# google-deepmind/dm_control

Hardware: AMD Instinct MI355X
Metric: env-steps/s (whole node) at batch 4096; max rel qpos error vs CPU (higher is better)
Workload: dtype f32

## Files before the change

### dm_control_amd/csrc/dmc_api.hip

```cpp
#include <hip/hip_runtime.h>
#include <dlfcn.h>

#include <cstdio>
#include <cstdlib>
#include <cstring>
#include <algorithm>
#include <string>
#include <type_traits>
#include <vector>

#include "../../include/dmc_batch.h"
#include "step_kernel.hip.h"
#include "step_tables.h"

namespace dmc {
hipError_t launch_step_f32(const LaunchGeom& g, hipStream_t stream, const StepLayout* d_layout, const StepOpts<float>& o,
                           const int* g_mi, const float* g_mr, const int* g_mc, const StepIO<float>& io, int nstep, int legacy, int mode, int outmask, int nsub);
hipError_t launch_step_f64(const LaunchGeom& g, hipStream_t stream, const StepLayout* d_layout, const StepOpts<double>& o,
                           const int* g_mi, const double* g_mr, const int* g_mc, const StepIO<double>& io, int nstep, int legacy, int mode, int outmask, int nsub);
}

using namespace dmc;

static thread_local std::string g_err;
// ... 257 lines not shown
      if (step_tables_build(&def, m->hm, nconmax, njmax, &err, njcon, -1)) {
        StepTables keep = b->tb; LaunchGeom kg = b->geom;
        b->tb = def;
        const bool def_fits = choose_geometry(b, lanes_per_env) == 0;
        if (fits && (!def_fits || b->geom.static_id < 0)) { b->tb = keep; b->geom = kg; }
      } else if (!fits) return fail(err);
    }
  }
  if (choose_geometry(b, lanes_per_env)) return -1;
  const StepLayout& L = b->tb.L;
  const StepDims& d = L.d;
  if (dev_alloc(b, &b->d_mi, (size_t)L.n_mi * sizeof(int), false, "") || dev_alloc(b, &b->d_mc, b->tb.mc.size() * sizeof(int), false, "") ||
      dev_alloc(b, &b->d_mr, (size_t)L.n_mr * b->elem, false, "") || dev_alloc(b, &b->d_layout, sizeof(StepLayout), false, "", &L)) return -2;
  if (upload_tables(b)) return -2;
  b->tb.opts.g_mr = b->d_mr;
  if (d.nslip) {
    if (dev_alloc(b, &b->d_ns_A, (size_t)b->B * d.nslip * d.nslip * b->elem, false, "noslip matrix")) return -2;
    b->tb.opts.ns_A = b->d_ns_A;
  }
  const int one = 1;
  if (dev_alloc(b, &b->d_epoch, sizeof(int), false, "stash epoch", &one)) return -2;
  if (dev_alloc(b, &b->d_work, 32 * 9 * sizeof(int), true, "work queue")) return -2;
  if (!getenv("DMC_NO_KSTASH") && !d.nmocap) {
    const size_t nk = (size_t)d.nq + d.nv + (L.s_qM - L.s_xpos);
    if (dev_alloc(b, &b->d_kstash, (size_t)b->B * nk * b->elem, false, "kinematic stash") ||
        dev_alloc(b, &b->d_kstash_i, (size_t)b->B * sizeof(int), true, "kinematic stash")) return -2;
  }
  if (b->geom.queue) {
    const int nit = (b->B * b->geom.lpe + 63) / 64;
    b->nxcd = getenv("DMC_XCDS") ? std::max(1, std::min(8, atoi(getenv("DMC_XCDS")))) : (b->ncu == 256 ? 8 : 1);
    if (b->geom.grid < 8 * b->nxcd) b->nxcd = 1;
    const bool one_l2_per_queue = b->nxcd > 1 || b->ncu <= 40 || getenv("DMC_XCDS");
    b->max_slices = getenv("DMC_SLICES") ? atoi(getenv("DMC_SLICES")) : (one_l2_per_queue ? 8 : 1);
    auto hw = [&](int n) { return b->precision == 64 ? n : (n + 1) / 2; };
    b->hand_n = hw(d.nq) + 2 * hw(d.nv) + hw(d.na) + 1;
    if (dev_alloc(b, &b->d_prog, (size_t)nit * sizeof(int), true, "piece counters") ||
        dev_alloc(b, &b->d_hand, (size_t)b->B * b->hand_n * sizeof(unsigned long long), false, "piece counters")) return -2;
  }
  if (b->geom.queue && !getenv("DMC_NO_LPT")) {
    b->nitems = (b->B * b->geom.lpe + 63) / 64;
    if (dev_alloc(b, &b->d_cost, (size_t)b->nitems * sizeof(int), true, "schedule") ||
        dev_alloc(b, &b->d_order, (size_t)b->nitems * sizeof(int), false, "schedule")) return -2;
    b->lpt = 1;
  }
  if (L.n_gs) {
    if (dev_alloc(b, &b->d_gscr, (size_t)b->B * L.n_gs * b->elem, true, "global scratch")) return -2;
    b->tb.opts.gscr = b->d_gscr;
// ... 101 lines not shown
    typedef int (*fn_t)(const LaunchGeom*, void*, const StepLayout*, const StepOpts<T>*, const int*, const T*, const int*, const StepIO<T>*, int, int, int, int, int);
    e = (hipError_t)((fn_t)b->spec_launch)(&b->geom, stream, b->d_layout, o, b->d_mi, (const T*)b->d_mr, b->d_mc, &io, nstep, legacy, mode, b->outmask, nsub);
  } else if constexpr (f64) e = launch_step_f64(b->geom, (hipStream_t)stream, b->d_layout, *o, b->d_mi, (const T*)b->d_mr, b->d_mc, io, nstep, legacy, mode, b->outmask, nsub);
  else e = launch_step_f32(b->geom, (hipStream_t)stream, b->d_layout, *o, b->d_mi, (const T*)b->d_mr, b->d_mc, io, nstep, legacy, mode, b->outmask, nsub);
  if (e != hipSuccess) return fail(std::string("kernel launch: ") + hipGetErrorString(e), -2);
  return 0;
}
static int launch_untimed(dmc_batch* b, int nstep, int legacy, LaunchMode mode, void* stream, const SeqArgs* sq) {
  HIP_TRY(hipSetDevice(b->device));
  b->launched_mask = b->outmask;
  return b->precision == 64 ? launch_t<double>(b, nstep, legacy, mode, stream, sq) : launch_t<float>(b, nstep, legacy, mode, stream, sq);
}
static int launch(dmc_batch* b, int nstep, int legacy, LaunchMode mode, void* stream, const SeqArgs* sq = nullptr) {
  HIP_TRY(hipSetDevice(b->device));
  TimerPair t;
  const bool timed = prof_begin(b, (hipStream_t)stream, &t);
  const int rc = launch_untimed(b, nstep, legacy, mode, stream, sq);
  const bool fwd = mode == MODE_FORWARD || mode == MODE_FORWARD_NOACT;
  if (timed) prof_end(b, (hipStream_t)stream, t, fwd ? 1 : 0,
                      mode == MODE_STEP ? nstep : mode == MODE_ROLLOUT ? nstep * (sq ? sq->nsub : 1) : mode == MODE_STEP1 ? 0 : 1);
  return rc;
}

extern "C" int dmc_batch_attach_specialised(dmc_batch* b, const char* so_path) {
  if (!b || !so_path) return fail("null argument");
  void* h = dlopen(so_path, RTLD_NOW | RTLD_LOCAL);
  if (!h) return fail(std::string("cannot load ") + so_path + ": " + dlerror());
  typedef const StepLayout* (*layout_t)();
  typedef void (*info_t)(int*);
  layout_t fl = (layout_t)dlsym(h, "dmc_spec_layout");
  info_t fi = (info_t)dlsym(h, "dmc_spec_info");
  void* launch = dlsym(h, "dmc_spec_launch");
  if (!fl || !fi || !launch) { dlclose(h); return fail("not a specialisation plugin (dmc_spec_* symbols missing)"); }
  int info[8]; fi(info);
  if (info[4] != b->precision) { dlclose(h); return fail("the plugin was built for another precision"); }
  const int so = b->precision == 64 ? (int)sizeof(StepOpts<double>) : (int)sizeof(StepOpts<float>);
  const int sio = b->precision == 64 ? (int)sizeof(StepIO<double>) : (int)sizeof(StepIO<float>);
  if (info[0] != (int)sizeof(StepLayout) || info[1] != so || info[2] != sio || info[3] != DMC_MODEL_VERSION || info[7] != (int)sizeof(LaunchGeom)) {
    dlclose(h); return fail("the plugin was built from other sources than this library (struct sizes / model version differ)");
  }
  if (info[5] != b->geom.lpe) { dlclose(h); return fail("the plugin was built for another lanes-per-environment shape"); }
  if (memcmp(fl(), &b->tb.L, sizeof(StepLayout)) != 0) { dlclose(h); return fail("the plugin's layout is not this batch's (another model or other caps)"); }
  if (b->spec_so) dlclose(b->spec_so);
  b->spec_so = h; b->spec_launch = launch; b->spec_features = info[6];
  typedef int (*tb_t)();
  tb_t tb = (tb_t)dlsym(h, "dmc_spec_task_args_bytes");
  b->spec_task_bytes = tb ? tb() : 0;
  b->task_on = 0;
  return 0;
}

extern "C" int dmc_batch_set_task_args(dmc_batch* b, const void* args, int nbytes) {
  if (!b || !args) return fail("null argument");
  if (!b->spec_task_bytes) return fail("the batch's kernel carries no task epilogue (attach a plugin built with a task header)");
  if (nbytes != b->spec_task_bytes) return fail("task argument block: size differs from the one the kernel was generated with");
  HIP_TRY(hipSetDevice(b->device));
  if (!b->d_task_args && dev_alloc(b, &b->d_task_args, (size_t)nbytes, false, "task arguments")) return -2;
  HIP_TRY(hipMemcpy(b->d_task_args, args, (size_t)nbytes, hipMemcpyHostToDevice));
  return 0;
}
extern "C" int dmc_batch_enable_task(dmc_batch* b, int on) {
  if (!b) return fail("null batch");
  if (on && (!b->spec_task_bytes || !b->d_task_args)) return fail("no task epilogue to enable (dmc_batch_set_task_args first)");
  b->task_on = on ? 1 : 0;
  return 0;
}

extern "C" int dmc_batch_step(dmc_batch* b, int nstep, int legacy_step, void* hip_stream) {
  if (!b) return fail("null batch");
  if (nstep < 1) return fail("nstep must be >= 1");
  if (legacy_step == 2 && b->tb.opts.integrator == DMC_INT_RK4) return fail("legacy_step 2 (step + mj_forward) is not implemented for RK4 models");
  return launch(b, nstep, legacy_step == 2 ? 2 : (legacy_step ? 1 : 0), MODE_STEP, hip_stream);
// ... 1091 lines not shown
```

### dm_control_amd/csrc/step_core.h

```cpp
#pragma once
#include "../../include/dmc_model_layout.h"
#include "step_layout.h"
#include "step_defs.h"
#include "step_math.h"
#include "step_lanes.h"
#include "step_dense.h"
#include "step_geom.h"

namespace dmc {
#ifdef DMC_HOST_EMU
inline int& emu_split_solves() { static int n = 0; return n; }
inline long long* emu_ls_counts() { static long long n[6] = {0, 0, 0, 0, 0, 0}; return n; }
inline long long* emu_ls_passes() { static long long n[3] = {0, 0, 0}; return n; }
#endif

#if defined(DMC_PROFILE) && !defined(DMC_HOST_EMU)
#define DMC_PROF(id) do { if (lane == 0) { const int t_ = (int)__builtin_readcyclecounter(); SI(prof)[id] += t_ - SI(prof)[33]; SI(prof)[33] = t_; } } while (0)
#else
#define DMC_PROF(id) ((void)0)
#endif
#ifdef DMC_TRACE_SUB
#define DMC_TSUB(region, cond, row) do { if (DMC_TRACE_SUB == (region) && (cond)) sub_stamp(row); } while (0)
#else
#define DMC_TSUB(region, cond, row) ((void)0)
// ... 225 lines not shown
      else __hip_atomic_store((unsigned*)(io.ctrl + (size_t)i*B + env), __float_as_uint((float)S(ctrl)[i]), __ATOMIC_RELAXED, __HIP_MEMORY_SCOPE_AGENT);
    }
  }
  DMC_DEV void load_handoff(const StepIO<T>& io, int env) {
    env = late(env);
    const int nq = L.d.nq, nv = L.d.nv, na = L.d.na, B = io.B;
    const u64h* h = io.hand + (size_t)env * io.hand_n;
    hand_get(S(qpos), h, nq); h += hand_words(nq);
    hand_get(S(qvel), h, nv); h += hand_words(nv);
    hand_get(S(qacc_warmstart), h, nv); h += hand_words(nv);
    if (na) { hand_get(S(act), h, na); h += hand_words(na); FOR_LANES(i, na) S(act_dot)[i] = 0; }
    { const u64h w = __hip_atomic_load(h, __ATOMIC_RELAXED, __HIP_MEMORY_SCOPE_AGENT); double t; __builtin_memcpy(&t, &w, 8); time_ = t; }
    FOR_LANES(i, nv) S(qfrc_applied)[i] = io.qfrc_applied ? io.qfrc_applied[(size_t)i*B + env] : (T)0;
    FOR_LANES(i, L.d.nu) {
      if (sizeof(T) == 8) { const u64h w = __hip_atomic_load((const u64h*)(io.ctrl + (size_t)i*B + env), __ATOMIC_RELAXED, __HIP_MEMORY_SCOPE_AGENT); T v; __builtin_memcpy(&v, &w, 8); S(ctrl)[i] = v; }
      else S(ctrl)[i] = (T)__uint_as_float(__hip_atomic_load((const unsigned*)(io.ctrl + (size_t)i*B + env), __ATOMIC_RELAXED, __HIP_MEMORY_SCOPE_AGENT));
    }
  }
#else
  DMC_DEV void store_handoff(const StepIO<T>&, int) {}
  DMC_DEV void load_handoff(const StepIO<T>&, int) {}
#endif
  DMC_DEV int kin_count() const { return L.s_qM - L.s_xpos; }
  DMC_DEV bool load_kstash(const StepIO<T>& io, int env) {
    env = late(env);
    if (io.kstash_i[env] != get_epoch()) return false;
    const int nq = L.d.nq, nv = L.d.nv, nk = kin_count();
    const T* h = io.kstash + (size_t)env*(nq + nv + nk);
    int bad = 0;
    FOR_LANES(i, nq) if (!(h[i] == S(qpos)[i])) bad = 1;
    FOR_LANES(i, nv) if (!(h[nq + i] == S(qvel)[i])) bad = 1;
    if (group_max<LPE>(bad)) return false;
    FOR_LANES(i, nk) S(xpos)[i] = h[nq + nv + i];
    DMC_WSYNC();
    kstash_env_geoms();
    return true;
  }
  DMC_DEV void store_kstash(const StepIO<T>& io, int env) {
    env = late(env);
    const int nq = L.d.nq, nv = L.d.nv, nk = kin_count();
    DMC_GLB T* h = G(io.kstash) + (size_t)env*(nq + nv + nk);
    FOR_LANES(i, nq) h[i] = S(qpos)[i];
    FOR_LANES(i, nv) h[nq + i] = S(qvel)[i];
    FOR_LANES(i, nk) h[nq + nv + i] = S(xpos)[i];
    if (lane == 0) G(io.kstash_i)[env] = get_epoch();
  }
  static constexpr bool kFeat = LS::kNV <= 0 || DMC_STATIC_FEATURES;
  static constexpr bool kSlices = LS::kNV <= 0 || LS::kNV > 16;
  static constexpr int kPFKin = LS::kNKin > 0 ? ((LS::kNKin + LPE - 1) / LPE < 24 ? (LS::kNKin + LPE - 1) / LPE : 24) : 0;
  struct Entry { int em, fast, kvalid, epoch; };
  struct EntryRegs {
    T qpos, qvel, warm, qfrc, ctrl, act, kq, kv;
    int ktag, epoch;
    T kd[kPFKin ? kPFKin : 1];
  };
  DMC_DEV static bool kstash_applies(const StepOpts<T>& o, const StepIO<T>& io, int mode, int legacy) {
    return io.kstash && mode == 0 && legacy && o.integrator != DMC_INT_RK4 && !io.stash_r;
  }
  DMC_DEV static void entry_issue(const StepLayout& L, const StepOpts<T>& o, const StepIO<T>& io, int env, int lane, int mode,
                                  int legacy, Entry* e, EntryRegs* r) {
    e->em = io.env_mode ? io.env_mode[env] : 0;
    e->kvalid = 0;
    e->epoch = *io.epoch;
#ifdef DMC_HOST_EMU
    e->fast = 0;
#else
    e->fast = (L.d.nq <= LPE && L.d.nv <= LPE && L.d.nu <= LPE && L.d.na <= LPE && !io.stash_r) ? 1 : 0;
#endif
    r->ktag = 0; r->epoch = 1;
    if (!e->fast) return;
    const size_t B = (size_t)io.B;
    const int nq = L.d.nq, nv = L.d.nv;
    r->qpos = lane < nq ? G(io.qpos)[lane*B + env] : (T)0;
    r->qvel = lane < nv ? G(io.qvel)[lane*B + env] : (T)0;
    r->warm = lane < nv ? G(io.qacc_warmstart)[lane*B + env] : (T)0;
    r->qfrc = (io.qfrc_applied && lane < nv) ? G(io.qfrc_applied)[lane*B + env] : (T)0;
    r->ctrl = lane < L.d.nu ? G(io.ctrl)[lane*B + env] : (T)0;
    r->act = (L.d.na && lane < L.d.na) ? G(io.act)[lane*B + env] : (T)0;
    if (!kstash_applies(o, io, mode, legacy)) return;
    r->ktag = G(io.kstash_i)[env]; r->epoch = e->epoch;
    const int nk = L.s_qM - L.s_xpos;
    const DMC_GLB T* h = G(io.kstash) + (size_t)env*(nq + nv + nk);
    r->kq = lane < nq ? h[lane] : (T)0;
    r->kv = lane < nv ? h[nq + lane] : (T)0;
#pragma unroll
    for (int k = 0; k < kPFKin; k++) { const int i = lane + k*LPE; r->kd[k] = i < nk ? h[nq + nv + i] : (T)0; }
  }
  DMC_DEV static void entry_commit(const StepLayout& L, const StepIO<T>& io, int env, int lane, Entry* e, const EntryRegs& r, T* s) {
    if (!e->fast) return;
    const int nq = L.d.nq, nv = L.d.nv;
    if (lane < nq) s[L.s_qpos + lane] = r.qpos;
    if (lane < nv) { s[L.s_qvel + lane] = r.qvel; s[L.s_qacc_warmstart + lane] = r.warm; s[L.s_qfrc_applied + lane] = r.qfrc; }
    if (lane < L.d.nu) s[L.s_ctrl + lane] = r.ctrl;
    if (L.d.na && lane < L.d.na) s[L.s_act + lane] = r.act;
    if (r.ktag != r.epoch) return;
    const int bad = ((lane < nq && !(r.kq == r.qpos)) || (lane < nv && !(r.kv == r.qvel))) ? 1 : 0;
    if (group_max<LPE>(bad)) return;
    const int nk = L.s_qM - L.s_xpos;
#pragma unroll
    for (int k = 0; k < kPFKin; k++) { const int i = lane + k*LPE; if (i < nk) s[L.s_xpos + i] = r.kd[k]; }
    if (kPFKin*LPE < nk) {
      const T* h = io.kstash + (size_t)env*(nq + nv + nk) + nq + nv;
      for (int i = lane + kPFKin*LPE; i < nk; i += LPE) s[L.s_xpos + i] = h[i];
    }
    e->kvalid = 1;
  }
  DMC_DEV void kstash_env_geoms() {
    if (!o.eg_n) return;
    FOR_LANES(g, L.d.ngeom) {
      const int k = o.eg_slot[g];
      if (k < 0) continue;
      const T* eg = (const T*)o.eg_data + (size_t)16*k*o.eg_B + SI(imisc)[IM_ENV];
      for (int j = 0; j < 3; j++) S(geom_xpos)[3*g + j] = eg[(size_t)j*o.eg_B];
      for (int j = 0; j < 9; j++) SG(geom_xmat)[9*g + j] = eg[(size_t)(3 + j)*o.eg_B];
    }
    DMC_WSYNC();
  }
  DMC_DEV void load_state(const StepIO<T>& io, int env, bool have_stash, const Entry& en, bool from_hand = false) {
    const int B = io.B;
    if (kSlices && from_hand) load_handoff(io, env);
    else if (en.fast) {
      if (L.d.na && lane < L.d.na) S(act_dot)[lane] = 0;
      time_ = io.time[env];
    } else {
      FOR_LANES(i, L.d.nq) S(qpos)[i] = io.qpos[(size_t)i*B + env];
      FOR_LANES(i, L.d.nv) {
        S(qvel)[i] = io.qvel[(size_t)i*B + env];
// ... 4 lines not shown
      if (L.d.na) FOR_LANES(i, L.d.na) { S(act)[i] = io.act[(size_t)i*B + env]; S(act_dot)[i] = 0; }
      time_ = io.time[env];
    }
    if (lane == 0) SI(imisc)[IM_ENV] = env;
    if (have_stash) {
      if (LPE >= 16) { if (lane < DMC_NWARNING) SI(imisc)[IM_WARN + lane] = 0; } else if (lane == 0) for (int k = 0; k < DMC_NWARNING; k++) SI(imisc)[IM_WARN + k] = 0;
      DMC_WSYNC();
      return;
    }
    if (lane == 0) {
      for (int k = 0; k < DMC_NWARNING; k++) SI(imisc)[IM_WARN + k] = 0;
      SI(imisc)[IM_NCON] = 0; SI(imisc)[IM_NEFC] = 0; SI(imisc)[IM_ITER] = 0;
      T* xp = S(xpos); T* xq = SG(xquat); T* xm = S(xmat); T* xi = S(xipos);
      xp[0] = xp[1] = xp[2] = 0; xi[0] = xi[1] = xi[2] = 0;
      xq[0] = 1; xq[1] = xq[2] = xq[3] = 0;
      for (int k = 0; k < 9; k++) xm[k] = (k % 4 == 0) ? (T)1 : (T)0;
      for (int k = 0; k < 10; k++) SG(cinert)[k] = 0;
      for (int k = 0; k < 6; k++) S(cvel)[k] = 0;
    }
    if (!L.d.msparse) FOR_LANES(i, L.d.nv * L.d.nv) S(qM)[i] = 0;
    FOR_LANES(i, L.d.nsensordata) S(sensordata)[i] = 0;
    DMC_WSYNC();
  }
  DMC_DEV void store_state(const StepIO<T>& io, int env) {
    env = late(env);
    const int B = io.B;
    FOR_LANES(i, L.d.nq) G(io.qpos)[(size_t)i*B + env] = S(qpos)[i];
    FOR_LANES(i, L.d.nv) {
      G(io.qvel)[(size_t)i*B + env] = S(qvel)[i];
      G(io.qacc_warmstart)[(size_t)i*B + env] = S(qacc_warmstart)[i];
    }
    if (L.d.na) FOR_LANES(i, L.d.na) G(io.act)[(size_t)i*B + env] = S(act)[i];
    if (lane == 0) G(io.time)[env] = time_;
#ifndef DMC_HOST_EMU
    if (LPE >= 16) { if (lane < DMC_NWARNING) { const int w = SI(imisc)[IM_WARN + lane]; if (w) atomicAdd(io.warning + (size_t)lane*B + env, w); } }
    else if (lane == 0) for (int k = 0; k < DMC_NWARNING; k++) if (SI(imisc)[IM_WARN + k]) atomicAdd(io.warning + (size_t)k*B + env, SI(imisc)[IM_WARN + k]);
#else
    if (lane == 0) for (int k = 0; k < DMC_NWARNING; k++) if (SI(imisc)[IM_WARN + k]) G(io.warning)[(size_t)k*B + env] += SI(imisc)[IM_WARN + k];
#endif
    if (SI(imisc)[IM_WARN + DMC_WARN_BADCTRL]) FOR_LANES(i, L.d.nu) io.ctrl[(size_t)i*B + env] = S(ctrl)[i];
  }
  DMC_DEV void store_outputs(const StepIO<T>& io, int env, int mask) {
    env = late(env);
    const int B = io.B;
    const int nb = L.d.nbody;
    if (mask & OUT_SENSOR) FOR_LANES(i, L.d.nsensordata) G(io.sensordata)[(size_t)i*B + env] = S(sensordata)[i];
    if (mask & OUT_XPOS) FOR_LANES(i, 3*nb) G(io.xpos)[(size_t)i*B + env] = S(xpos)[i];
    if (mask & OUT_XQUAT) FOR_LANES(i, 4*nb) G(io.xquat)[(size_t)i*B + env] = SG(xquat)[i];
    if (mask & OUT_XMAT) FOR_LANES(i, 9*nb) G(io.xmat)[(size_t)i*B + env] = S(xmat)[i];
    if (mask & OUT_XIPOS) FOR_LANES(i, 3*nb) io.xipos[(size_t)i*B + env] = S(xipos)[i];
    if (mask & OUT_SUBTREE_COM) FOR_LANES(i, 3*nb) G(io.subtree_com)[(size_t)i*B + env] = S(subtree_com)[i];
    if (mask & OUT_GEOM) {
      FOR_LANES(i, 3*L.d.ngeom) io.geom_xpos[(size_t)i*B + env] = S(geom_xpos)[i];
      FOR_LANES(i, 9*L.d.ngeom) io.geom_xmat[(size_t)i*B + env] = SG(geom_xmat)[i];
    }
    if (mask & OUT_SITE) FOR_LANES(sid, L.d.nsite) {
// ... 4195 lines not shown
        if (it == 0 && stage == 0) trace_stamp(io, env, 4); else if (trailing) trace_stamp(io, env, 7);
        if (mode == 3 && stage == 0 && it > 0 && it % nsub == 0) store_seq(io, env, it / nsub - 1);
        if (mode == 0 && stage == 0 && it >= 1) probe_store(io, env, it - 1, 1);
        if (trailing && !fwd_after) break;
        call_acc(mode == 2, stage > 0 || !sens_acc, stepping && !trailing && nstage == 1);
        if (trailing) break;
        if (it == 0 && stage == 0) trace_stamp(io, env, 5);
        if (stage == 0 && stepping && !retried && bad_acc()) {
          if (lane == 0) SI(imisc)[IM_WARN + DMC_WARN_BADQACC]++;
          if (!(o.disableflags & DMC_DSBL_AUTORESET)) { DMC_WSYNC(); reset_state(); retried = 1; continue; }
        }
        if (stage == 0 && stepping && it == ntotal - 1) { dump_debug(io, env); if (mode == 0 && !legacy) store_outputs(io, env, outmask); }
        if (nstage > 1) rk4_stage(stage);
        stage++;
      }
      if (!stepping || trailing) break;
      if (nstage > 1) rk4_finish(); else call_euler();
      if (it == 0) trace_stamp(io, env, 6);
      DMC_PROF(PROF_EULER);
    }
    if constexpr (kSlices) if (!last_piece) { store_handoff(io, env); DMC_PROF(PROF_STORE); prof_end(io, env); return; }
    if (!stepping) dump_debug(io, env);
    if (!stepping && launch_mode == 0) probe_store(io, env, 0, nstep);
    if (!stepping || legacy || mode == 3) { DMC_PROF(PROF_TRAIL); store_outputs(io, env, outmask); }
    if (stash) store_stash(io, env, mode == 0 && legacy && !fwd_after);
    if (io.kstash && mode == 0 && legacy && o.integrator != DMC_INT_RK4) store_kstash(io, env);
    store_state(io, env);
    DMC_PROF(PROF_STORE);
    prof_end(io, env);
  }
#undef MI
#undef MR
#undef GC
#undef S
#undef SG
#undef SI
#undef FOR_LANES
};


#ifndef DMC_HOST_EMU
template <typename T, int LPE, typename LS>
struct StageFns {
  typedef StepCore<T, LPE, LS> Core;
  static DMC_FN void posvel(LS ls, const DMC_LDS StepOpts<T>* o, DMC_LDS int* mi, DMC_LDS T* mr, const int* gc, DMC_LDS T* s,
                            DMC_LDS int* si, int lane, int flags, int outmask) {
    Core c(ls, *(const StepOpts<T>*)o, (const int*)mi, (const T*)mr, gc, (T*)s, (int*)si, lane);
    c.stage_posvel(flags & 1, outmask, flags & 2, flags & 4);
  }
  static DMC_FN void acc(LS ls, const DMC_LDS StepOpts<T>* o, DMC_LDS int* mi, DMC_LDS T* mr, const int* gc, DMC_LDS T* s,
// ... 21 lines not shown
```

### dm_control_amd/csrc/step_kernel.hip.h

```cpp
#pragma once
#include <hip/hip_runtime.h>

#include "step_core.h"
#ifdef DMC_TASK_HEADER
#define DMC_TASK_IN_KERNEL 1
#include DMC_TASK_HEADER
#endif

namespace dmc {

struct LaunchGeom {
  int lpe;
  int waves;
  int envs_per_block;
  int lds_bytes;
  int grid;
  int queue;
  int blocks_per_cu;
  int static_id;
};

#ifndef DMC_MIN_WAVES
#define DMC_MIN_WAVES 2
#endif
#ifndef DMC_MAX_THREADS
#define DMC_MAX_THREADS 320
#endif

#if defined(DMC_LAYOUTS_HEADER)
#include DMC_LAYOUTS_HEADER
#elif defined(DMC_PROFILE) && __has_include("static_layouts_prof.gen.h")
#include "static_layouts_prof.gen.h"
#elif __has_include("static_layouts.gen.h")
#include "static_layouts.gen.h"
#endif
#ifndef DMC_NSTATIC
#define DMC_NSTATIC 0
#endif

template <typename T> constexpr int stepopts_lds_bytes() { return (int)((sizeof(StepOpts<T>) + 15) / 16 * 16); }
template <typename T> constexpr int opts_lds_bytes() { return stepopts_lds_bytes<T>() + (int)((sizeof(StepIO<T>) + 15) / 16 * 16); }

template <typename T, int LPE, typename LS, bool QUEUE>
__device__ __forceinline__ void step_kernel_body(LS ls, const StepOpts<T>& o_arg, const int* __restrict__ g_mi,
                                                 const T* __restrict__ g_mr, const int* __restrict__ g_mc, const StepIO<T>& io_arg, int nstep, int legacy,
                                                 int mode, int outmask, int nsub) {
  extern __shared__ __attribute__((aligned(16))) unsigned char smem[];
  const StepLayout& L = ls.get();
  StepOpts<T>* o_lds = reinterpret_cast<StepOpts<T>*>(smem);
  unsigned char* tables = smem + opts_lds_bytes<T>();
  int* mi = reinterpret_cast<int*>(tables);
  T* mr = reinterpret_cast<T*>(tables + (size_t)L.n_mi * sizeof(int));
  const int tid = threadIdx.x, nthr = blockDim.x;
  const int t_entry = io_arg.trace ? (int)(wall_clock64() & 0x7fffffffll) : 0;
  typedef StepCore<T, LPE, LS> Core;
  constexpr int epw = 64 / LPE;
  const int nblk = gridDim.x, xcd = blockIdx.x & 7, q = nblk >> 3, r = nblk & 7;
  const int lblk = xcd * q + (xcd < r ? xcd : r) + (blockIdx.x >> 3);
  const int wave = __builtin_amdgcn_readfirstlane(tid >> 6), wpb = nthr >> 6;
  const int nitems = (io_arg.B + epw - 1) / epw, nwaves = nblk * wpb;
  const size_t tables_bytes = (size_t)L.n_mi * sizeof(int) + (size_t)L.n_mr_lds * sizeof(T) + (L.d.coldlds ? (size_t)L.n_mc * sizeof(int) : 0);
  const size_t env_bytes = (size_t)L.n_sr * sizeof(T) + (size_t)L.n_si * sizeof(int);
  typename Core::Entry en;
  typename Core::EntryRegs er;
  if (tid == 0) *o_lds = o_arg;
  StepIO<T>* io_lds = reinterpret_cast<StepIO<T>*>(smem + stepopts_lds_bytes<T>());
  if (tid == 64 % nthr) *io_lds = io_arg;
  const StepIO<T>& io = *io_lds;
  int* const q_work = QUEUE ? io_arg.work : nullptr;
  int* const q_prog = QUEUE ? io_arg.prog : nullptr;
  const int q_slices = QUEUE ? io_arg.slices : 0, q_nxcd = QUEUE ? io_arg.nxcd : 1;
  const int NX = (QUEUE && q_work && q_nxcd > 1) ? q_nxcd : 1;
  const int xq = NX > 1 ? (int)(__builtin_amdgcn_s_getreg(20 | (0 << 6) | (3 << 11)) % (unsigned)NX) : 0;
  const int nq_items = (nitems - xq + NX - 1) / NX;
  const int npieces = (Core::kSlices && QUEUE && q_work && q_prog && q_slices > 1 && mode == 0) ? q_slices : 1;
  const int nslots = nq_items * npieces;
  int* const head = (QUEUE && q_work) ? q_work + 32 * (1 + xq) : nullptr;
  int slot = lblk * wpb + wave, piece = 0;
  bool have_item = slot < nitems;
  if (QUEUE && head) {
    int nx = 0;
    if ((tid & 63) == 0) nx = atomicAdd(head, 1);
    nx = __builtin_amdgcn_readfirstlane(nx);
    have_item = nx < nslots;
    for (piece = 0; nx >= nq_items && piece < npieces - 1; piece++) nx -= nq_items;
    slot = nx * NX + xq;
  }
  int env0 = 0;
  if (have_item && piece == 0) {
    const int item = io_arg.order ? io_arg.order[slot] : slot;
    env0 = item * epw + ((tid / LPE) & (epw - 1));
    if (env0 >= io_arg.B) env0 = io_arg.B - 1;
    Core::entry_issue(L, o_arg, io_arg, env0, tid % LPE, mode, legacy, &en, &er);
  } else if (have_item) {
    const int item = io_arg.order ? io_arg.order[slot] : slot;
    int e0 = item * epw + ((tid / LPE) & (epw - 1));
    if (e0 >= io_arg.B) e0 = io_arg.B - 1;
    en.em = io_arg.env_mode ? io_arg.env_mode[e0] : 0; en.fast = 0; en.kvalid = 0; en.epoch = *io_arg.epoch;
  }
  for (int i = tid; i < L.n_mi; i += nthr) mi[i] = g_mi[i];
  for (int i = tid; i < L.n_mr_lds; i += nthr) mr[i] = g_mr[i];
  int* mc_lds = reinterpret_cast<int*>(tables + (size_t)L.n_mi * sizeof(int) + (size_t)L.n_mr_lds * sizeof(T));
  const size_t cold_bytes = L.d.coldlds ? (size_t)L.n_mc * sizeof(int) : 0;
  if (L.d.coldlds) for (int i = tid; i < L.n_mc; i += nthr) mc_lds[i] = g_mc[i];
  if (have_item && piece == 0) Core::entry_commit(L, io_arg, env0, tid % LPE, &en, er, reinterpret_cast<T*>(tables + tables_bytes + (size_t)(tid / LPE) * env_bytes));
  __syncthreads();
  if (have_item) for (;;) {
    int t = threadIdx.x;
    asm volatile("" : "+v"(t));
    const int g = t / LPE, lane = t % LPE;
    unsigned char* base = tables + (size_t)L.n_mi * sizeof(int) + (size_t)L.n_mr_lds * sizeof(T) + cold_bytes + (size_t)g * env_bytes;
    T* s = reinterpret_cast<T*>(base);
    int* si = reinterpret_cast<int*>(base + (size_t)L.n_sr * sizeof(T));
    StepCore<T, LPE, LS> core(ls, *o_lds, mi, mr, L.d.coldlds ? (const int*)mc_lds : g_mc, s, si, lane);
    const int item = io.order ? io.order[slot] : slot;
    const int env = item * epw + (g & (epw - 1));
    int* tr = io.trace ? io.trace + (size_t)(io.trace_slot & 7) * 8 * nitems : nullptr;
    const long long tw0 = tr ? (long long)wall_clock64() : 0;
    if (QUEUE && piece > 0)
      while (__hip_atomic_load(q_prog + item, __ATOMIC_RELAXED, __HIP_MEMORY_SCOPE_AGENT) < piece) __builtin_amdgcn_s_sleep(8);
    const long long tw1 = tr ? (long long)wall_clock64() : 0;
    const long long t0 = io.cost ? (long long)__builtin_readcyclecounter() : 0;
    if (tr && (threadIdx.x & 63) == 0 && piece == 0) { tr[item] = t_entry; tr[nitems + item] = (int)(wall_clock64() & 0x7fffffffll); }
    if (env < io.B) core.run(io, env, nstep, legacy, mode, outmask, nsub, en, piece, npieces);
#ifdef DMC_TASK_HEADER
    if (io.task_args && mode == 0 && piece == npieces - 1 && env < io.B) {
      if (dmc_task::kReadsGlobal) asm volatile("s_waitcnt vmcnt(0)" ::: "memory");
// ... 25 lines not shown
    nx = __builtin_amdgcn_readfirstlane(nx);
    if (nx >= nslots) break;
    for (piece = 0; nx >= nq_items && piece < npieces - 1; piece++) nx -= nq_items;
    slot = nx * NX + xq;
    const int nitem = io.order ? io.order[slot] : slot;
    int nenv = nitem * epw + ((threadIdx.x / LPE) & (epw - 1));
    if (nenv >= io.B) nenv = io.B - 1;
    en.em = io.env_mode ? io.env_mode[nenv] : 0; en.fast = 0; en.kvalid = 0;
  }
  if (QUEUE && q_work && (threadIdx.x & 63) == 0) {
    if (atomicAdd(q_work + 1, 1) == nwaves - 1) {
      atomicExch(q_work + 1, 0);
      for (int x = 0; x < NX; x++) atomicExch(q_work + 32 * (1 + x), 0);
      if (npieces > 1) for (int i = 0; i < nitems; i++) q_prog[i] = 0;
    }
  }
}

template <typename T, int LPE, bool QUEUE>
__global__ void __launch_bounds__(DMC_MAX_THREADS, DMC_MIN_WAVES)
step_kernel(const StepLayout* __restrict__ Lp, StepOpts<T> o, const int* __restrict__ g_mi, const T* __restrict__ g_mr,
            const int* __restrict__ g_mc, StepIO<T> io, int nstep, int legacy, int mode, int outmask, int nsub) {
  DynLayoutSrc ls; ls.p = Lp;
  step_kernel_body<T, LPE, DynLayoutSrc, QUEUE>(ls, o, g_mi, g_mr, g_mc, io, nstep, legacy, mode, outmask, nsub);
}

#if DMC_NSTATIC > 0
template <int SID> struct StaticLayout;
#define DMC_DEF_STATIC(ID)                                                            \
  static __device__ const StepLayout kStaticLayout##ID = DMC_STATIC_LAYOUT_##ID;     \
  template <> struct StaticLayout<ID> {                                               \
    static constexpr int kNV = DMC_STATIC_NV_##ID;    \
    static constexpr StepLayout kL = DMC_STATIC_LAYOUT_##ID;                                      \
    static constexpr int kJGlobal = kL.d.jglobal;    \
    static constexpr int kNKin = kL.s_qM - kL.s_xpos;          \
    static constexpr int kTreeMax = kL.d.treemax;    \
    static constexpr int kTreeUni = kL.d.treeuni;    \
    __device__ __forceinline__ const StepLayout& get() const { return kStaticLayout##ID; } \
  };
DMC_STATIC_IDS(DMC_DEF_STATIC)
#undef DMC_DEF_STATIC

template <typename T, int LPE, int SID, bool QUEUE>
__global__ void __launch_bounds__(DMC_MAX_THREADS, DMC_MIN_WAVES)
step_kernel_static(StepOpts<T> o, const int* __restrict__ g_mi, const T* __restrict__ g_mr,
                   const int* __restrict__ g_mc, StepIO<T> io, int nstep, int legacy, int mode, int outmask, int nsub) {
  step_kernel_body<T, LPE, StaticLayout<SID>, QUEUE>(StaticLayout<SID>(), o, g_mi, g_mr, g_mc, io, nstep, legacy, mode, outmask, nsub);
}
#endif

template <typename T>
static hipError_t launch_step_t(const LaunchGeom& g, hipStream_t stream, const StepLayout* d_layout, const StepOpts<T>& o,
                                const int* g_mi, const T* g_mr, const int* g_mc, const StepIO<T>& io, int nstep, int legacy, int mode, int outmask, int nsub) {
  const dim3 grid(g.grid), block(g.waves * 64);
#define DMC_LAUNCH_Q(LPE, Q)                                                                                    \
  {                                                                                                             \
    hipError_t e = hipFuncSetAttribute(reinterpret_cast<const void*>(&step_kernel<T, LPE, Q>),                  \
                                       hipFuncAttributeMaxDynamicSharedMemorySize, g.lds_bytes);                \
    if (e != hipSuccess) return e;                                                                              \
    hipLaunchKernelGGL((step_kernel<T, LPE, Q>), grid, block, g.lds_bytes, stream, d_layout, o, g_mi, g_mr, g_mc, io, nstep, \
                       legacy, mode, outmask, nsub);                                                                  \
  }
#define DMC_LAUNCH(LPE) { if (io.work) DMC_LAUNCH_Q(LPE, true) else DMC_LAUNCH_Q(LPE, false) }
#define DMC_LAUNCH_STATIC_Q(LPE, SID, Q)                                                                        \
  {                                                                                                             \
    hipError_t e = hipFuncSetAttribute(reinterpret_cast<const void*>(&step_kernel_static<T, LPE, SID, Q>),      \
                                       hipFuncAttributeMaxDynamicSharedMemorySize, g.lds_bytes);                \
    if (e != hipSuccess) return e;                                                                              \
    hipLaunchKernelGGL((step_kernel_static<T, LPE, SID, Q>), grid, block, g.lds_bytes, stream, o, g_mi, g_mr, g_mc, io,  \
                       nstep, legacy, mode, outmask, nsub);                                                           \
// ... 33 lines not shown
```

### dm_control_amd/csrc/step_layout.h

```cpp
#pragma once
#include <stdint.h>

#define DMC_JGLOBAL_LEVEL(nv) ((nv) > 48 ? 3 : ((nv) > 32 ? 2 : ((nv) > 16 ? 1 : 0)))

struct StepDims {
  int nq, nv, nu, nbody, njnt, ngeom, nsite, nsensor, nsensordata, npair;
  int nlevel;
  int nchild;
  int nM;
  int nconmax;
  int njmax;
  int rk4;
  int ntri;
  int elliptic;
  int nfric;
  int ncyl;
  int ncylx;
  int ntendon, nwrap;
  int fluid;
  int nstv;
  int nlimten;
  int nlimball;
  int neq;
  int neqrow;
// ... 188 lines not shown
#define X(name, cnt) int mi_##name;
  STEP_MODEL_INT_TABLES(X)
#undef X
#define X(name, cnt) int mr_##name;
  STEP_MODEL_REAL_TABLES(X)
#undef X
#define X(name, cnt) int mc_##name;
  STEP_MODEL_COLD_TABLES(X)
#undef X
#define X(name, cnt) int s_##name;
  STEP_SCRATCH_ALL_REAL(X)
#undef X
#define X(name, cnt) int si_##name;
  STEP_SCRATCH_INT(X)
#undef X
  int n_mi, n_mr, n_mc;
  int n_mr_lds;
  int n_sr, n_si;
  int n_keep;
  int n_gs, gs_Jc, gs_LM, gs_M, gs_cf;
  int gs_xquat, gs_geom_xmat, gs_cinert, gs_cdof_dot;
};

template <typename T>
struct StepOpts {
  T timestep, gravity[3], impratio, tolerance, ls_tolerance, meaninertia, density, viscosity, noslip_tolerance;
  int integrator, cone, iterations, ls_iterations, disableflags, noslip_iterations;
  int any_damping;
  int islands;
  double timestep_d;
  const void* eg_data; const int* eg_slot; int eg_n, eg_B;
  void* ns_A;
  const void* xfrc; int xfrc_B;
  const void* mocap_pos; const void* mocap_quat; int mocap_B;
  void* gscr;
  const void* g_mr;
};

static inline void step_layout_build(StepLayout* L, const StepDims& d) {
  L->d = d;
  int o = 0;
#define X(name, cnt) L->mi_##name = o; o += (cnt);
  STEP_MODEL_INT_TABLES(X)
#undef X
  L->n_mi = (o + 3) & ~3;
  o = 0;
// ... 84 lines not shown
```

Baseline: 81.65 million.

## Use 16-byte vector I/O for kinematic stash, table staging and kernel args

Pads each env's kinematic stash record so the kinematic block shares the alignment of the LDS xpos offset. This lets the stash prefetch, commit and store paths use 16-byte vector loads and stores. Table staging into LDS is rewritten as batched 16-byte loads, and kernel arguments are read straight from the kernarg segment into registers and then written to LDS. The final state store is specialised for single-pass lanes, with the time written separately. The aim is to cut per-env memory instructions in launch prologues and epilogues. In exchange it adds padding, alignment assumptions on table sizes and the kernarg layout, and an epoch bump when a plugin is attached.

After: 82.70 million (median of 6 runs). 1.01x the previous value.

```diff
diff --git a/dm_control_amd/csrc/dmc_api.hip b/dm_control_amd/csrc/dmc_api.hip
--- a/dm_control_amd/csrc/dmc_api.hip
+++ b/dm_control_amd/csrc/dmc_api.hip
@@ -303,7 +303,7 @@
   if (dev_alloc(b, &b->d_epoch, sizeof(int), false, "stash epoch", &one)) return -2;
   if (dev_alloc(b, &b->d_work, 32 * 9 * sizeof(int), true, "work queue")) return -2;
   if (!getenv("DMC_NO_KSTASH") && !d.nmocap) {
-    const size_t nk = (size_t)d.nq + d.nv + (L.s_qM - L.s_xpos);
+    const size_t nk = (size_t)kstash_record(d.nq, d.nv, L.s_qM - L.s_xpos, L.s_xpos, (int)b->elem).stride;
     if (dev_alloc(b, &b->d_kstash, (size_t)b->B * nk * b->elem, false, "kinematic stash") ||
         dev_alloc(b, &b->d_kstash_i, (size_t)b->B * sizeof(int), true, "kinematic stash")) return -2;
   }
@@ -451,6 +451,7 @@
   return rc;
 }
 
+static int bump_epoch(dmc_batch* b, hipStream_t stream, bool wait);
 extern "C" int dmc_batch_attach_specialised(dmc_batch* b, const char* so_path) {
   if (!b || !so_path) return fail("null argument");
   void* h = dlopen(so_path, RTLD_NOW | RTLD_LOCAL);
@@ -476,7 +477,7 @@
   tb_t tb = (tb_t)dlsym(h, "dmc_spec_task_args_bytes");
   b->spec_task_bytes = tb ? tb() : 0;
   b->task_on = 0;
-  return 0;
+  return bump_epoch(b, 0, true);
 }
 
 extern "C" int dmc_batch_set_task_args(dmc_batch* b, const void* args, int nbytes) {
diff --git a/dm_control_amd/csrc/step_core.h b/dm_control_amd/csrc/step_core.h
--- a/dm_control_amd/csrc/step_core.h
+++ b/dm_control_amd/csrc/step_core.h
@@ -271,16 +271,28 @@
   DMC_DEV void load_handoff(const StepIO<T>&, int) {}
 #endif
   DMC_DEV int kin_count() const { return L.s_qM - L.s_xpos; }
+#if defined(DMC_NO_WIDE_IO) || defined(DMC_HOST_EMU)
+  static constexpr bool kWideIO = false;
+#else
+  static constexpr bool kWideIO = true;
+  typedef T TV __attribute__((ext_vector_type(16 / sizeof(T))));
+#endif
+  static constexpr int kE = 16 / (int)sizeof(T);
+  DMC_DEV static KStashRecord krec(const StepLayout& L) {
+    const int head = L.d.nq + L.d.nv, nk = L.s_qM - L.s_xpos;
+    return kWideIO ? kstash_record(L.d.nq, L.d.nv, nk, L.s_xpos, (int)sizeof(T)) : KStashRecord{head, head + nk};
+  }
   DMC_DEV bool load_kstash(const StepIO<T>& io, int env) {
     env = late(env);
     if (io.kstash_i[env] != get_epoch()) return false;
     const int nq = L.d.nq, nv = L.d.nv, nk = kin_count();
-    const T* h = io.kstash + (size_t)env*(nq + nv + nk);
+    const KStashRecord kr = krec(L);
+    const T* h = io.kstash + (size_t)env*kr.stride;
     int bad = 0;
     FOR_LANES(i, nq) if (!(h[i] == S(qpos)[i])) bad = 1;
     FOR_LANES(i, nv) if (!(h[nq + i] == S(qvel)[i])) bad = 1;
     if (group_max<LPE>(bad)) return false;
-    FOR_LANES(i, nk) S(xpos)[i] = h[nq + nv + i];
+    FOR_LANES(i, nk) S(xpos)[i] = h[kr.kin + i];
     DMC_WSYNC();
     kstash_env_geoms();
     return true;
@@ -288,20 +300,52 @@
   DMC_DEV void store_kstash(const StepIO<T>& io, int env) {
     env = late(env);
     const int nq = L.d.nq, nv = L.d.nv, nk = kin_count();
-    DMC_GLB T* h = G(io.kstash) + (size_t)env*(nq + nv + nk);
+    const KStashRecord kr = krec(L);
+    DMC_GLB T* h = G(io.kstash) + (size_t)env*kr.stride;
+#if !defined(DMC_NO_WIDE_IO) && !defined(DMC_HOST_EMU)
+    {
+      const int pad = kr.kin % kE, a = pad ? (kE - pad < nk ? kE - pad : nk) : 0, nf = (nk - a) / kE, b = a + nf*kE;
+      const TV* sv = reinterpret_cast<const TV*>(S(xpos) + a);
+      DMC_GLB TV* hv = reinterpret_cast<DMC_GLB TV*>(h + kr.kin + a);
+      if constexpr (LS::kNKin > 0) {
+        constexpr int trips = (LS::kNKin / kE + LPE - 1) / LPE;
+        TV v[trips];
+        if (nf > 0) {
+#pragma unroll
+          for (int k = 0; k < trips; k++) { const int j = lane + k*LPE; v[k] = sv[j < nf ? j : nf - 1]; }
+#pragma unroll
+          for (int k = 0; k < trips; k++) { const int j = lane + k*LPE; if (j < nf) hv[j] = v[k]; }
+        }
+      } else {
+        for (int j = lane; j < nf; j += LPE) hv[j] = sv[j];
+      }
+      FOR_LANES(i, nq) h[i] = S(qpos)[i];
+      FOR_LANES(i, nv) h[nq + i] = S(qvel)[i];
+      FOR_LANES(i, a) h[kr.kin + i] = S(xpos)[i];
+      for (int i = b + lane; i < nk; i += LPE) h[kr.kin + i] = S(xpos)[i];
+      if (lane == 0) G(io.kstash_i)[env] = get_epoch();
+      return;
+    }
+#endif
     FOR_LANES(i, nq) h[i] = S(qpos)[i];
     FOR_LANES(i, nv) h[nq + i] = S(qvel)[i];
-    FOR_LANES(i, nk) h[nq + nv + i] = S(xpos)[i];
+    FOR_LANES(i, nk) h[kr.kin + i] = S(xpos)[i];
     if (lane == 0) G(io.kstash_i)[env] = get_epoch();
   }
   static constexpr bool kFeat = LS::kNV <= 0 || DMC_STATIC_FEATURES;
   static constexpr bool kSlices = LS::kNV <= 0 || LS::kNV > 16;
   static constexpr int kPFKin = LS::kNKin > 0 ? ((LS::kNKin + LPE - 1) / LPE < 24 ? (LS::kNKin + LPE - 1) / LPE : 24) : 0;
+  static constexpr int kNCh = LS::kNKin > 0 ? (LS::kNKin + 2*kE - 2) / kE : 0;
+  static constexpr int kPFCh = kNCh ? ((kNCh + LPE - 1) / LPE < 24 / kE ? (kNCh + LPE - 1) / LPE : 24 / kE) : 0;
   struct Entry { int em, fast, kvalid, epoch; };
   struct EntryRegs {
     T qpos, qvel, warm, qfrc, ctrl, act, kq, kv;
     int ktag, epoch;
+#if defined(DMC_NO_WIDE_IO) || defined(DMC_HOST_EMU)
     T kd[kPFKin ? kPFKin : 1];
+#else
+    TV kc[kPFCh ? kPFCh : 1];
+#endif
   };
   DMC_DEV static bool kstash_applies(const StepOpts<T>& o, const StepIO<T>& io, int mode, int legacy) {
     return io.kstash && mode == 0 && legacy && o.integrator != DMC_INT_RK4 && !io.stash_r;
@@ -329,11 +373,19 @@
     if (!kstash_applies(o, io, mode, legacy)) return;
     r->ktag = G(io.kstash_i)[env]; r->epoch = e->epoch;
     const int nk = L.s_qM - L.s_xpos;
-    const DMC_GLB T* h = G(io.kstash) + (size_t)env*(nq + nv + nk);
+    const KStashRecord kr = krec(L);
+    const DMC_GLB T* h = G(io.kstash) + (size_t)env*kr.stride;
     r->kq = lane < nq ? h[lane] : (T)0;
     r->kv = lane < nv ? h[nq + lane] : (T)0;
-#pragma unroll
-    for (int k = 0; k < kPFKin; k++) { const int i = lane + k*LPE; r->kd[k] = i < nk ? h[nq + nv + i] : (T)0; }
+#if defined(DMC_NO_WIDE_IO) || defined(DMC_HOST_EMU)
+#pragma unroll
+    for (int k = 0; k < kPFKin; k++) { const int i = lane + k*LPE; r->kd[k] = i < nk ? h[kr.kin + i] : (T)0; }
+#else
+    const int pad = kr.kin % kE, nch = (pad + nk + kE - 1) / kE;
+    const DMC_GLB TV* hv = reinterpret_cast<const DMC_GLB TV*>(h + (kr.kin - pad));
+#pragma unroll
+    for (int k = 0; k < kPFCh; k++) { const int j = lane + k*LPE; r->kc[k] = hv[j < nch ? j : nch - 1]; }
+#endif
   }
   DMC_DEV static void entry_commit(const StepLayout& L, const StepIO<T>& io, int env, int lane, Entry* e, const EntryRegs& r, T* s) {
     if (!e->fast) return;
@@ -346,12 +398,32 @@
     const int bad = ((lane < nq && !(r.kq == r.qpos)) || (lane < nv && !(r.kv == r.qvel))) ? 1 : 0;
     if (group_max<LPE>(bad)) return;
     const int nk = L.s_qM - L.s_xpos;
+    const KStashRecord kr = krec(L);
+#if defined(DMC_NO_WIDE_IO) || defined(DMC_HOST_EMU)
 #pragma unroll
     for (int k = 0; k < kPFKin; k++) { const int i = lane + k*LPE; if (i < nk) s[L.s_xpos + i] = r.kd[k]; }
     if (kPFKin*LPE < nk) {
-      const T* h = io.kstash + (size_t)env*(nq + nv + nk) + nq + nv;
+      const T* h = io.kstash + (size_t)env*kr.stride + kr.kin;
       for (int i = lane + kPFKin*LPE; i < nk; i += LPE) s[L.s_xpos + i] = h[i];
     }
+#else
+    const int pad = kr.kin % kE, nch = (pad + nk + kE - 1) / kE;
+    TV* sv = reinterpret_cast<TV*>(s + (L.s_xpos - pad));
+#pragma unroll
+    for (int k = 0; k < kPFCh; k++) {
+      const int j = lane + k*LPE, lo = j*kE - pad;
+      if (j >= nch) continue;
+      if (lo >= 0 && lo + kE <= nk) sv[j] = r.kc[k];
+      else {
+#pragma unroll
+        for (int c = 0; c < kE; c++) if (lo + c >= 0 && lo + c < nk) s[L.s_xpos + lo + c] = r.kc[k][c];
+      }
+    }
+    if (kPFCh*LPE < nch) {
+      const T* h = io.kstash + (size_t)env*kr.stride + kr.kin;
+      for (int i = (kPFCh ? kPFCh*LPE*kE - pad : 0) + lane; i < nk; i += LPE) s[L.s_xpos + i] = h[i];
+    }
+#endif
     e->kvalid = 1;
   }
   DMC_DEV void kstash_env_geoms() {
@@ -402,16 +474,40 @@
     FOR_LANES(i, L.d.nsensordata) S(sensordata)[i] = 0;
     DMC_WSYNC();
   }
-  DMC_DEV void store_state(const StepIO<T>& io, int env) {
+  DMC_DEV void store_time(const StepIO<T>& io, int env) {
+    env = late(env);
+    if (lane == 0) G(io.time)[env] = time_;
+  }
+  DMC_DEV void store_state(const StepIO<T>& io, int env, bool time_stored = false) {
     env = late(env);
     const int B = io.B;
+#if !defined(DMC_NO_WIDE_IO) && !defined(DMC_HOST_EMU)
+    const int nq = L.d.nq, nv = L.d.nv, na = L.d.na;
+    if (nq <= LPE && nv <= LPE && na <= LPE && L.d.nu <= LPE) {
+      DMC_GLB T* const p_qpos = G(io.qpos); DMC_GLB T* const p_qvel = G(io.qvel); DMC_GLB T* const p_warm = G(io.qacc_warmstart);
+      DMC_GLB T* const p_act = G(io.act); DMC_GLB double* const p_time = G(io.time);
+      int* const p_warn = io.warning; T* const p_ctrl = io.ctrl;
+      const T v_qpos = lane < nq ? S(qpos)[lane] : (T)0, v_qvel = lane < nv ? S(qvel)[lane] : (T)0;
+      const T v_warm = lane < nv ? S(qacc_warmstart)[lane] : (T)0, v_act = (na && lane < na) ? S(act)[lane] : (T)0;
+      const int v_warn = (LPE >= 16 && lane < DMC_NWARNING) ? SI(imisc)[IM_WARN + lane] : 0;
+      const int badctrl = SI(imisc)[IM_WARN + DMC_WARN_BADCTRL];
+      if (!time_stored && lane == 0) p_time[env] = time_;
+      if (lane < nq) p_qpos[(size_t)lane*B + env] = v_qpos;
+      if (lane < nv) { p_qvel[(size_t)lane*B + env] = v_qvel; p_warm[(size_t)lane*B + env] = v_warm; }
+      if (na && lane < na) p_act[(size_t)lane*B + env] = v_act;
+      if (LPE >= 16) { if (lane < DMC_NWARNING && v_warn) atomicAdd(p_warn + (size_t)lane*B + env, v_warn); }
+      else if (lane == 0) for (int k = 0; k < DMC_NWARNING; k++) if (SI(imisc)[IM_WARN + k]) atomicAdd(p_warn + (size_t)k*B + env, SI(imisc)[IM_WARN + k]);
+      if (badctrl && lane < L.d.nu) p_ctrl[(size_t)lane*B + env] = S(ctrl)[lane];
+      return;
+    }
+#endif
     FOR_LANES(i, L.d.nq) G(io.qpos)[(size_t)i*B + env] = S(qpos)[i];
     FOR_LANES(i, L.d.nv) {
       G(io.qvel)[(size_t)i*B + env] = S(qvel)[i];
       G(io.qacc_warmstart)[(size_t)i*B + env] = S(qacc_warmstart)[i];
     }
     if (L.d.na) FOR_LANES(i, L.d.na) G(io.act)[(size_t)i*B + env] = S(act)[i];
-    if (lane == 0) G(io.time)[env] = time_;
+    if (!time_stored && lane == 0) G(io.time)[env] = time_;
 #ifndef DMC_HOST_EMU
     if (LPE >= 16) { if (lane < DMC_NWARNING) { const int w = SI(imisc)[IM_WARN + lane]; if (w) atomicAdd(io.warning + (size_t)lane*B + env, w); } }
     else if (lane == 0) for (int k = 0; k < DMC_NWARNING; k++) if (SI(imisc)[IM_WARN + k]) atomicAdd(io.warning + (size_t)k*B + env, SI(imisc)[IM_WARN + k]);
@@ -4653,10 +4749,11 @@
     if constexpr (kSlices) if (!last_piece) { store_handoff(io, env); DMC_PROF(PROF_STORE); prof_end(io, env); return; }
     if (!stepping) dump_debug(io, env);
     if (!stepping && launch_mode == 0) probe_store(io, env, 0, nstep);
+    if (kWideIO) store_time(io, env);
     if (!stepping || legacy || mode == 3) { DMC_PROF(PROF_TRAIL); store_outputs(io, env, outmask); }
     if (stash) store_stash(io, env, mode == 0 && legacy && !fwd_after);
     if (io.kstash && mode == 0 && legacy && o.integrator != DMC_INT_RK4) store_kstash(io, env);
-    store_state(io, env);
+    store_state(io, env, kWideIO);
     DMC_PROF(PROF_STORE);
     prof_end(io, env);
   }
diff --git a/dm_control_amd/csrc/step_kernel.hip.h b/dm_control_amd/csrc/step_kernel.hip.h
--- a/dm_control_amd/csrc/step_kernel.hip.h
+++ b/dm_control_amd/csrc/step_kernel.hip.h
@@ -41,7 +41,16 @@
 template <typename T> constexpr int stepopts_lds_bytes() { return (int)((sizeof(StepOpts<T>) + 15) / 16 * 16); }
 template <typename T> constexpr int opts_lds_bytes() { return stepopts_lds_bytes<T>() + (int)((sizeof(StepIO<T>) + 15) / 16 * 16); }
 
-template <typename T, int LPE, typename LS, bool QUEUE>
+#ifndef DMC_NO_WIDE_IO
+typedef unsigned int u32x4 __attribute__((ext_vector_type(4)));
+#define DMC_KARG __attribute__((address_space(4)))
+template <typename T> constexpr int kernarg_io_offset(int karg0) {
+  static_assert(alignof(StepOpts<T>) == 8 && alignof(StepIO<T>) == 8 && sizeof(StepOpts<T>) % 8 == 0 && sizeof(StepIO<T>) % 8 == 0, "kernel-argument layout");
+  return karg0 + (int)sizeof(StepOpts<T>) + 3 * (int)sizeof(void*);
+}
+#endif
+
+template <typename T, int LPE, typename LS, bool QUEUE, int KARG0>
 __device__ __forceinline__ void step_kernel_body(LS ls, const StepOpts<T>& o_arg, const int* __restrict__ g_mi,
                                                  const T* __restrict__ g_mr, const int* __restrict__ g_mc, const StepIO<T>& io_arg, int nstep, int legacy,
                                                  int mode, int outmask, int nsub) {
@@ -63,9 +72,28 @@
   const size_t env_bytes = (size_t)L.n_sr * sizeof(T) + (size_t)L.n_si * sizeof(int);
   typename Core::Entry en;
   typename Core::EntryRegs er;
+  StepIO<T>* io_lds = reinterpret_cast<StepIO<T>*>(smem + stepopts_lds_bytes<T>());
+#ifdef DMC_NO_WIDE_IO
   if (tid == 0) *o_lds = o_arg;
-  StepIO<T>* io_lds = reinterpret_cast<StepIO<T>*>(smem + stepopts_lds_bytes<T>());
   if (tid == 64 % nthr) *io_lds = io_arg;
+#else
+  constexpr int n_argo = (int)(sizeof(StepOpts<T>) / 4), n_arg = n_argo + (int)(sizeof(StepIO<T>) / 4);
+  constexpr int arg_trips = (n_arg + 63) / 64;
+  constexpr int io_off = kernarg_io_offset<T>(KARG0);
+  unsigned areg[arg_trips];
+  {
+    const DMC_KARG unsigned char* ka = (const DMC_KARG unsigned char*)__builtin_amdgcn_kernarg_segment_ptr();
+#pragma unroll
+    for (int k = 0; k < arg_trips; k++) {
+      areg[k] = 0;
+      if (k * nthr < n_arg) {
+        int d = tid + k * nthr;
+        d = d < n_arg ? d : n_arg - 1;
+        areg[k] = *(const DMC_KARG unsigned*)(ka + (d < n_argo ? KARG0 + 4 * d : io_off + 4 * (d - n_argo)));
+      }
+    }
+  }
+#endif
   const StepIO<T>& io = *io_lds;
   int* const q_work = QUEUE ? io_arg.work : nullptr;
   int* const q_prog = QUEUE ? io_arg.prog : nullptr;
@@ -98,11 +126,48 @@
     if (e0 >= io_arg.B) e0 = io_arg.B - 1;
     en.em = io_arg.env_mode ? io_arg.env_mode[e0] : 0; en.fast = 0; en.kvalid = 0; en.epoch = *io_arg.epoch;
   }
+  int* mc_lds = reinterpret_cast<int*>(tables + (size_t)L.n_mi * sizeof(int) + (size_t)L.n_mr_lds * sizeof(T));
+  const size_t cold_bytes = L.d.coldlds ? (size_t)L.n_mc * sizeof(int) : 0;
+#ifdef DMC_NO_WIDE_IO
   for (int i = tid; i < L.n_mi; i += nthr) mi[i] = g_mi[i];
   for (int i = tid; i < L.n_mr_lds; i += nthr) mr[i] = g_mr[i];
-  int* mc_lds = reinterpret_cast<int*>(tables + (size_t)L.n_mi * sizeof(int) + (size_t)L.n_mr_lds * sizeof(T));
-  const size_t cold_bytes = L.d.coldlds ? (size_t)L.n_mc * sizeof(int) : 0;
   if (L.d.coldlds) for (int i = tid; i < L.n_mc; i += nthr) mc_lds[i] = g_mc[i];
+#else
+  {
+    constexpr int kTableBatch = 4;
+    const int c_mi = L.n_mi / 4, c_mr = c_mi + (int)((size_t)L.n_mr_lds * sizeof(T) / 16);
+    const int c_all = c_mr + (L.d.coldlds ? L.n_mc / 4 : 0);
+    const unsigned long long a_mi = (unsigned long long)g_mi, a_mr = (unsigned long long)g_mr - 16ull * (unsigned)c_mi,
+                             a_mc = (unsigned long long)g_mc - 16ull * (unsigned)c_mr;
+    u32x4* dst = reinterpret_cast<u32x4*>(tables);
+    __builtin_assume(nthr >= 64);
+    auto batch = [&](int base) {
+      u32x4 treg[kTableBatch];
+#pragma unroll
+      for (int k = 0; k < kTableBatch; k++) {
+        if (base + k * nthr < c_all) {
+          int c = base + k * nthr + tid;
+          c = c < c_all ? c : c_all - 1;
+          const unsigned long long a = c < c_mi ? a_mi : (c < c_mr ? a_mr : a_mc);
+          treg[k] = *(const DMC_GLB u32x4*)(a + 16ull * (unsigned)c);
+        }
+      }
+#pragma unroll
+      for (int k = 0; k < kTableBatch; k++) {
+        const int c = base + k * nthr + tid;
+        if (c < c_all) dst[c] = treg[k];
+      }
+    };
+    batch(0);
+#pragma clang loop vectorize(disable) unroll(disable)
+    for (int base = kTableBatch * nthr; base < c_all; base += kTableBatch * nthr) batch(base);
+#pragma unroll
+    for (int k = 0; k < arg_trips; k++) {
+      const int d = tid + k * nthr;
+      if (d < n_arg) *reinterpret_cast<unsigned*>(smem + (d < n_argo ? 4 * d : stepopts_lds_bytes<T>() + 4 * (d - n_argo))) = areg[k];
+    }
+  }
+#endif
   if (have_item && piece == 0) Core::entry_commit(L, io_arg, env0, tid % LPE, &en, er, reinterpret_cast<T*>(tables + tables_bytes + (size_t)(tid / LPE) * env_bytes));
   __syncthreads();
   if (have_item) for (;;) {
@@ -174,7 +239,7 @@
 step_kernel(const StepLayout* __restrict__ Lp, StepOpts<T> o, const int* __restrict__ g_mi, const T* __restrict__ g_mr,
             const int* __restrict__ g_mc, StepIO<T> io, int nstep, int legacy, int mode, int outmask, int nsub) {
   DynLayoutSrc ls; ls.p = Lp;
-  step_kernel_body<T, LPE, DynLayoutSrc, QUEUE>(ls, o, g_mi, g_mr, g_mc, io, nstep, legacy, mode, outmask, nsub);
+  step_kernel_body<T, LPE, DynLayoutSrc, QUEUE, (int)sizeof(const StepLayout*)>(ls, o, g_mi, g_mr, g_mc, io, nstep, legacy, mode, outmask, nsub);
 }
 
 #if DMC_NSTATIC > 0
@@ -197,7 +262,7 @@
 __global__ void __launch_bounds__(DMC_MAX_THREADS, DMC_MIN_WAVES)
 step_kernel_static(StepOpts<T> o, const int* __restrict__ g_mi, const T* __restrict__ g_mr,
                    const int* __restrict__ g_mc, StepIO<T> io, int nstep, int legacy, int mode, int outmask, int nsub) {
-  step_kernel_body<T, LPE, StaticLayout<SID>, QUEUE>(StaticLayout<SID>(), o, g_mi, g_mr, g_mc, io, nstep, legacy, mode, outmask, nsub);
+  step_kernel_body<T, LPE, StaticLayout<SID>, QUEUE, 0>(StaticLayout<SID>(), o, g_mi, g_mr, g_mc, io, nstep, legacy, mode, outmask, nsub);
 }
 #endif
 
diff --git a/dm_control_amd/csrc/step_layout.h b/dm_control_amd/csrc/step_layout.h
--- a/dm_control_amd/csrc/step_layout.h
+++ b/dm_control_amd/csrc/step_layout.h
@@ -234,6 +234,13 @@
   int gs_xquat, gs_geom_xmat, gs_cinert, gs_cdof_dot;
 };
 
+struct KStashRecord { int kin, stride; };
+constexpr KStashRecord kstash_record(int nq, int nv, int nk, int s_xpos, int elem) {
+  const int e = 16 / elem, head = nq + nv;
+  const int kin = head + ((s_xpos - head) % e + e) % e;
+  return KStashRecord{kin, (kin + nk + e - 1) / e * e};
+}
+
 template <typename T>
 struct StepOpts {
   T timestep, gravity[3], impratio, tolerance, ls_tolerance, meaninertia, density, viscosity, noslip_tolerance;
```
